# devmentality/LEAStereo

Measured on AMD Instinct MI355X. Metric: stereo pairs/s at 576×960 D=192, 1/2/4/8 GPU; EPE vs reference, higher is better.
Workload: dtype f32; 1 GPU; SceneFlow 576x960 D=192 fp32, batch 1 per GPU (BASELINE configs[1]); height=576, width=960, maxdisp=192, global_batch=1, parallelism=dp1 (pairs sharded over ranks, no collective in the step), launch=hip graph replay

## Files before the change

include/leastereo_hip_tuning.h:

```cpp
#ifndef LEASTEREO_HIP_TUNING_H
#define LEASTEREO_HIP_TUNING_H

#ifdef __cplusplus
extern "C" {
#endif

int lea_conv3d_set_tile_override(int nt, int tw, int td);

int lea_conv3d_set_rs_gather(int on);

int lea_conv1x1_set_vector(int on);

int lea_conv3d_bf16_set_tile_override(int th, int td, int mt);

int lea_conv3d_bf16_set_variant(int variant);

int lea_conv3d_bf16_set_stream1x1(int on);

int lea_conv3d_bf16_set_pair_split(int on);

int lea_resample_bf16_set_batch(int k);

int lea_resample_bf16_set_cols(int on);

int lea_resample_set_mode(int mode);

int lea_conv2d_set_small(int on);

const char* lea_conv2d_kernel_name_cin(int B, int cin, int cout, int H, int W);

int lea_disparity_set_register_form(int on);

int lea_tapsum_set_rows(int on);

int lea_staged_rows(int Hi, int Ho, int ac, int R, int halo);

int lea_conv3d_wino_set_w22(int on);

int lea_conv3d_wino_set_tile_override(int np, int td, int f);

int lea_conv3d_wino_set_variant(int variant);

int lea_conv3d_wino2_set_walk(int spw);

int lea_conv3d_wino2_set_halo16(int on);

int lea_conv3d_wino2_set_lane_halo16(int on);

int lea_conv3d_wino_set_fence(int on);

int lea_conv3d_wino2_set_pipeline(int on);

int lea_conv3d_wino2p_set_wpre(int on);

int lea_conv3d_wino44_set(int on);

int lea_conv3d_wino44_set_upre(int on);

int lea_conv3d_wino44_set_sched(int s);

int lea_conv3d_wino44_set_group(int g);

int lea_conv3d_wino_set_epi_buf(int on);

int lea_conv3d_wino_set_small_cout(int mode);

int lea_conv3d_wino_set_block48(int on);

int lea_rectify_set_tile(int mode);

#ifdef __cplusplus
}
#endif
#endif
```

leastereo_amd/_lib.py:

```python
from __future__ import annotations

import ctypes
import os
import threading

LIB_PATH = os.environ.get(
    "LEASTEREO_HIP_LIB",
    os.path.join(os.path.dirname(os.path.abspath(__file__)), "libleastereo_hip.so"))

ABI_VERSION = 14
LEA_F32 = 0
LEA_BF16 = 1
LEA_RELU = 1
LEA_RESIDUAL = 2
LEA_PAIR_SUM = 4
LEA_CVS_TMAJOR = 8
LEA_E_INVALID = 1001

_p = ctypes.c_void_p
_i = ctypes.c_int
_i64 = ctypes.c_int64
_u = ctypes.c_uint

SIGNATURES = {
# ... 69 lines not shown
    "lea_resample_bf16_set_batch": (_i, [_i]),
    "lea_resample_bf16_set_cols": (_i, [_i]),
    "lea_conv3d_wino_set_w22": (_i, [_i]),
    "lea_conv3d_bf16_set_pair_split": (_i, [_i]),
    "lea_disparity_set_register_form": (_i, [_i]),
    "lea_tapsum_set_rows": (_i, [_i]),
    "lea_staged_rows": (_i, [_i, _i, _i, _i, _i]),
    "lea_conv1x1_resampled_bf16": (_i, [_p, _i64, _i, _i, _i, _p, _p, _p, _p, _i64, _i, _i, _i, _i, _i,
                                        _i, _u, _p]),
    "lea_to_c8_bf16": (_i, [_p, _i64, _p, _i64, _i, _i, _i64, _p]),
    "lea_conv2d_packed_elems_bf16": (ctypes.c_size_t, [_i, _i]),
    "lea_conv2d_pack_weights_bf16": (_i, [_p, _p, _i, _i, _p]),
    "lea_conv2d_bnrelu_bf16": (_i, [_p, _i64, _p, _p, _p, _p, _i64, _p, _i64, _i, _i, _i, _i, _i,
                                    _u, _p]),
    "lea_from_c8_bf16": (_i, [_p, _i64, _p, _i64, _i, _i, _i64, _p]),
    "lea_conv3d_wino_packed_floats": (ctypes.c_size_t, [_i, _i]),
    "lea_conv3d_wino_pack_weights": (_i, [_p, _p, _i, _i, _p]),
    "lea_conv3d_bnrelu_wino": (_i, [_p, _i64, _p, _i64, _i, _p, _p, _p, _p, _i64, _p, _i64,
                                    _i, _i, _i, _i, _i, _i, _u, _i, _p]),
    "lea_conv3d_bnrelu_costvolume_wino": (_i, [_p, _p, _i64, _p, _p, _p, _p, _i64, _i, _i, _i,
                                               _i, _i, _i, _u, _i, _p]),
    "lea_conv3d_wino_kernel_name": (ctypes.c_char_p, [_i, _i, _i, _i, _i, _i, _i]),
    "lea_conv3d_wino_down2_supported": (_i, [_i, _i, _i, _i, _i, _i]),
    "lea_conv3d_wino_down2_kernel_name": (ctypes.c_char_p, [_i, _i, _i, _i, _i, _i]),
    "lea_conv3d_bnrelu_wino_down2": (_i, [_p, _i64, _p, _p, _p, _p, _i64, _i, _i, _i, _i, _i, _i, _u, _i, _p]),
    "lea_conv3d_wino_down2_cat_supported": (_i, [_i, _i, _i, _i, _i, _i, _i]),
    "lea_conv3d_wino_down2_cat_kernel_name": (ctypes.c_char_p, [_i, _i, _i, _i, _i, _i, _i]),
    "lea_conv3d_bnrelu_wino_down2_cat": (_i, [_p, _i64, _p, _i64, _i, _p, _p, _p, _p, _i64, _i, _i, _i, _i, _i, _i,
                                              _u, _i, _p]),
    "lea_conv3d_wino_dp_down2_supported": (_i, [_i, _i, _i, _i, _i, _i]),
    "lea_conv3d_wino_dp_down2_kernel_name": (ctypes.c_char_p, [_i, _i, _i, _i, _i, _i, _i]),
    "lea_conv3d_bnrelu_wino_dp_down2": (_i, [_p, _i64, _p, _p, _p, _p, _i64, _p, _i64, _p, _i64, _i, _i, _i, _i, _i,
                                             _i, _u, _i, _p]),
    "lea_resample3d_down2_supported": (_i, [_i, _i, _i, _i, _i, _i, _i]),
    "lea_resample3d_trilinear_down2": (_i, [_p, _i64, _p, _i64, _p, _i64, _i, _i, _i, _i, _i, _i, _i, _i, _p, _p,
                                            _u, _i, _p]),
    "lea_conv3d_wino_set_tile_override": (_i, [_i, _i, _i]),
    "lea_conv3d_wino_set_variant": (_i, [_i]),
    "lea_conv3d_wino2_set_walk": (_i, [_i]),
    "lea_conv3d_wino2_set_halo16": (_i, [_i]),
    "lea_conv3d_wino2_set_lane_halo16": (_i, [_i]),
    "lea_conv3d_wino_set_fence": (_i, [_i]),
    "lea_resample_set_mode": (_i, [_i]),
    "lea_conv2d_set_small": (_i, [_i]),
    "lea_conv2d_kernel_name_cin": (ctypes.c_char_p, [_i, _i, _i, _i, _i]),
    "lea_conv2d_bnrelu_pair": (_i, [_p, _i64, _p, _p, _p, _p, _i64, _p, _i64, _p, _i64, _i, _i, _i, _i, _i,
                                    _i, _u, _p]),
    "lea_conv3d_wino2_set_pipeline": (_i, [_i]),
    "lea_conv3d_wino2p_set_wpre": (_i, [_i]),
    "lea_conv3d_wino44_set": (_i, [_i]),
    "lea_conv3d_wino44_set_upre": (_i, [_i]),
    "lea_conv3d_wino44_set_sched": (_i, [_i]),
    "lea_conv3d_wino44_set_group": (_i, [_i]),
    "lea_conv3d_wino_set_epi_buf": (_i, [_i]),
    "lea_conv3d_set_rs_gather": (_i, [_i]),
    "lea_conv1x1_set_vector": (_i, [_i]),
    "lea_conv3d_bf16_set_stream1x1": (_i, [_i]),
    "lea_conv3d_wino_set_small_cout": (_i, [_i]),
    "lea_conv3d_wino_set_block48": (_i, [_i]),
    "lea_cv_stem_split_weights": (_i, [_p, _p, _p, _i, _i, _p]),
    "lea_cv_stem_combine": (_i, [_p, _i64, _p, _i64, _p, _p, _p, _i64, _i, _i, _i, _i, _i, _u, _i,
                                 _p]),
    "lea_cv_stem_map_windows": (_i, [_i, _i, ctypes.POINTER(_i), ctypes.POINTER(_i)]),
    "lea_conv2d_windowed_tiles": (_i, [_i, _i, _i, _i, _i, ctypes.POINTER(_i)]),
    "lea_conv2d_bnrelu_windowed": (_i, [_p, _i64, _p, _p, _p, _p, _i64, _i, _i, _i, _i, _i, _i, _i, _i, _i, _i,
                                        _u, _i, _p]),
    "lea_cv_stem_down2_supported": (_i, [_i, _i, _i, _i, _i]),
    "lea_cv_stem_combine_down2": (_i, [_p, _i64, _p, _i64, _p, _p, _p, _i64, _p, _i64, _i, _i, _i, _i, _i,
                                       _u, _i, _p]),
    "lea_standardize_workspace_bytes": (ctypes.c_size_t, [_i]),
    "lea_standardize_crop_u8": (_i, [_p, _p, _i, _i, _i, _i, _p, _p, _i, _i, _p, _p]),
    "lea_train_transform_workspace_bytes": (ctypes.c_size_t, [_i]),
    "lea_train_transform_u8": (_i, [_p, _p, _i, _i, _i, _i, _p, _p, _p, _p, _p, _p, _i, _i,
                                    ctypes.c_float, _p, _p, _p]),
    "lea_standardize_tiles_workspace_bytes": (ctypes.c_size_t, []),
    "lea_standardize_tiles_u8": (_i, [_p, _p, _i, _i, _i, _p, _i, _p, _p, _i, _i, _p, _p]),
    "lea_tile_blend_f32": (_i, [_p, _i64, _p, _i, _p, _i, _i, _i, _i, _i, _i, _i, _i, _p, _i, _i, _p, _p]),
    "lea_disparity_metrics_workspace_bytes": (ctypes.c_size_t, [_i, _i, _i]),
    "lea_disparity_metrics": (_i, [_p, _i64, _p, _i64, _i, _i, _i, ctypes.c_float, _i, _i,
                                   _i, _i, _i, _p, _p, _p, _p]),
    "lea_conv3d_wgrad_workspace_bytes": (ctypes.c_size_t, [_i, _i, _i, _i, _i, _i, _i]),
    "lea_conv3d_wgrad": (_i, [_p, _p, _p, _p, ctypes.c_size_t, _i, _i, _i, _i, _i, _i, _i, _p]),
    "lea_conv2d_wgrad_workspace_bytes": (ctypes.c_size_t, [_i, _i, _i, _i, _i]),
    "lea_conv2d_wgrad": (_i, [_p, _p, _p, _p, ctypes.c_size_t, _i, _i, _i, _i, _i, _p]),
    "lea_conv2d_s3_backward_data": (_i, [_p, _p, _p, _i, _i, _i, _i, _i, _p]),
    "lea_conv2d_s3_wgrad_workspace_bytes": (ctypes.c_size_t, [_i, _i, _i, _i, _i]),
    "lea_conv2d_s3_wgrad": (_i, [_p, _p, _p, _p, ctypes.c_size_t, _i, _i, _i, _i, _i, _p]),
    "lea_conv3d_flip_weights": (_i, [_p, _p, _i, _i, _i, _p]),
    "lea_bn_workspace_bytes": (ctypes.c_size_t, [_i]),
    "lea_bn_forward_f32": (_i, [_p, _p, _i, _i, _i64, _p, _p, _p, _p, ctypes.c_float, ctypes.c_float,
                                _i, _u, _p, _p, _p, _p]),
    "lea_bn_backward_f32": (_i, [_p, _p, _p, _p, _i, _i, _i64, _p, _p, _p, _i, _u, _p, _p, _p, _p]),
    "lea_disparity_regression_backward": (_i, [_p, _p, _p, _p, _i, _i, _i, _i, _i, _p]),
    "lea_build_cost_volume_backward": (_i, [_p, _p, _p, _i, _i, _i, _i, _i, _p]),
    "lea_resample3d_backward_workspace_bytes": (ctypes.c_size_t, [_i, _i, _i, _i, _i, _i, _i, _i]),
    "lea_resample3d_trilinear_backward": (_i, [_p, _p, _p, ctypes.c_size_t, _i, _i, _i, _i, _i, _i, _i, _i,
                                               _i, _p]),
}

_lib = None
_lock = threading.Lock()


class HipKernelError(RuntimeError):
    pass


def load():
    global _lib
    if _lib is not None:
        return _lib
    with _lock:
        if _lib is None:
            if not os.path.exists(LIB_PATH):
                raise HipKernelError(
                    f"{LIB_PATH} not found: build it with `make` (hipcc --offload-arch=gfx950); "
                    "the LEAStereo hot path has no fallback")
            lib = ctypes.CDLL(LIB_PATH)
            for name, (res, args) in SIGNATURES.items():
                fn = getattr(lib, name)
                fn.restype = res
                fn.argtypes = args
            _apply_env_tuning(lib)
            _lib = lib
    return _lib


TUNING_ENV = {"LEASTEREO_WINO2_WALK": "lea_conv3d_wino2_set_walk",
              "LEASTEREO_HALO16": "lea_conv3d_wino2_set_halo16",
              "LEASTEREO_LANE_HALO16": "lea_conv3d_wino2_set_lane_halo16",
              "LEASTEREO_WINO_FENCE": "lea_conv3d_wino_set_fence",
              "LEASTEREO_RESAMPLE_MODE": "lea_resample_set_mode",
              "LEASTEREO_CONV2D_SMALL": "lea_conv2d_set_small",
              "LEASTEREO_WINO2_PIPE": "lea_conv3d_wino2_set_pipeline",
              "LEASTEREO_WINO2P_WPRE": "lea_conv3d_wino2p_set_wpre",
              "LEASTEREO_WINO44": "lea_conv3d_wino44_set",
              "LEASTEREO_WINO44_UPRE": "lea_conv3d_wino44_set_upre",
              "LEASTEREO_EPI_BUF": "lea_conv3d_wino_set_epi_buf",
              "LEASTEREO_RS_GATHER": "lea_conv3d_set_rs_gather",
              "LEASTEREO_1X1_VEC": "lea_conv1x1_set_vector",
              "LEASTEREO_BF16_1X1": "lea_conv3d_bf16_set_stream1x1",
              "LEASTEREO_RESAMPLE_K": "lea_resample_bf16_set_batch",
              "LEASTEREO_RESAMPLE_COLS": "lea_resample_bf16_set_cols",
              "LEASTEREO_W22": "lea_conv3d_wino_set_w22",
              "LEASTEREO_PAIR_SPLIT": "lea_conv3d_bf16_set_pair_split",
              "LEASTEREO_DISP_REG": "lea_disparity_set_register_form",
              "LEASTEREO_TAPSUM_ROWS": "lea_tapsum_set_rows"}


def _apply_env_tuning(lib):
    for var, fn in TUNING_ENV.items():
        if os.environ.get(var):
            if getattr(lib, fn)(int(os.environ[var])) != 0:
                raise HipKernelError(f"{var}={os.environ[var]}: {lib.lea_last_error().decode()}")


def check(rc: int, what: str):
    if rc != 0:
        msg = load().lea_last_error().decode(errors="replace")
        raise HipKernelError(f"{what} failed (rc={rc}): {msg}")
```

leastereo_amd/csrc/conv3d_wino.hip:

```cpp
#include "wino_common.h"

namespace lea {
namespace wino {

template <int F, int Q, int MT, int NP, int TD, bool H16 = false>
struct Cfg {
  static constexpr bool DP = MT == 0;
  static constexpr int MTE = DP ? 1 : MT;
  static constexpr int TDA = DP ? 1 : TD;
  static constexpr int NSTEP = DP ? 12 : 9;
  static_assert(!DP || TD == 2, "a depth-paired tile covers two output planes");
  static constexpr int NX = F + 2;
  static constexpr int COP = 16 * MTE;
  static constexpr bool SWZ = (COP % 32) == 0;
  static constexpr int RPG = 16 / Q;
  static constexpr int TW = F * Q;
  static constexpr int TH = 4 * NP * RPG;
  static constexpr int RH = TH + 2, RW = TW + 2;
  static constexpr int PLANE = RH * RW;
  static constexpr int PLANES = TD + 2;
  static constexpr int IMG = PLANES * PLANE;
  static constexpr int XSLOTS = (IMG + 63) / 64;
  static constexpr int CIS = conflict_free_cis<F, Q>(64 * XSLOTS, RW);
  static constexpr int RWA = TW + 8;
  static constexpr int PLANEA = RH * RWA;
  static constexpr int IMGA = PLANES * PLANEA;
  static constexpr int BLK16 = IMGA / 4;
  static constexpr int PIECES16 = (BLK16 + 63) / 64;
  static constexpr int cb2(int c) {
    int base = 1;
    for (int k = 1; k <= c; ++k) {
      const int want = (k & 1 ? 2 : 0) + (k & 2 ? 32 : 0) + 1, lo = base + IMGA;
      base = lo + ((want - lo) % 64 + 64) % 64;
    }
    return base;
  }
  static_assert(!H16 || (Q == 16 && F == 4), "16-byte halo: one tile row per lane group");
  static constexpr int CSH = PIECES16 * 256;
  static constexpr int cbh(int c) { return 1 + c * CSH; }
  static_assert(!H16 || (CSH % 64 == 0 && RWA % 4 == 0 && PLANEA % 4 == 0), "b128 halo map");
  static constexpr int XS = H16 ? (cbh(CIN_B) + 3) / 4 * 4 : CIN_B * CIS;
  static constexpr int RWX = H16 ? RWA : RW;
  static constexpr int PLX = H16 ? PLANEA : PLANE;
  static constexpr int WS = NSTEP * 3 * CIN_B * COP;
  static constexpr int WSLOTS = (WS + 255) / 256;
  static constexpr int STAGE = XS + 256 * WSLOTS;
  static_assert(XS % 4 == 0 && WS % 4 == 0 && RW % 2 == 0 && PLANE % 2 == 0, "aligned LDS regions and b64 reads");
  static_assert(2 * STAGE * 4 * 2 <= 160 * 1024, "two double-buffered workgroups per CU");
};

constexpr int kDownXch = 4 * 64 * 4;
__device__ __forceinline__ float lerp_dp(float l0, float v0, float l1, float v1) {
// ... 895 lines not shown
    wino::g_override[0] = 0;
    return 0;
  }
  LEA_CHECK_ARG((np == 1 || np == 2) && (td == 1 || td == 2) && (f == 0 || f == 2 || f == 4 || f == 8),
                "lea_conv3d_wino_set_tile_override: bad tile np=%d td=%d f=%d", np, td, f);
  wino::g_override[0] = np;
  wino::g_override[1] = td;
  wino::g_override[2] = f;
  return 0;
}

extern "C" int lea_conv3d_wino_set_block48(int on) {
  clear_error();
  LEA_CHECK_ARG(on == 0 || on == 1, "lea_conv3d_wino_set_block48: on=%d", on);
  wino::g_block48 = on;
  return 0;
}

extern "C" int lea_conv3d_wino_set_epi_buf(int on) {
  clear_error();
  LEA_CHECK_ARG(on == 0 || on == 1, "lea_conv3d_wino_set_epi_buf: on=%d", on);
  wino::g_epibuf = on;
  return 0;
}

extern "C" int lea_conv3d_wino_set_small_cout(int mode) {
  clear_error();
  LEA_CHECK_ARG(mode == 0 || mode == 1, "lea_conv3d_wino_set_small_cout: mode=%d", mode);
  wino::g_small16 = mode;
  return 0;
}

extern "C" int lea_conv3d_wino2_set_pipeline(int on) {
  clear_error();
  LEA_CHECK_ARG(on == 0 || on == 1, "lea_conv3d_wino2_set_pipeline: on=%d", on);
  wino::g_pipe = on;
  return 0;
}

extern "C" int lea_conv3d_wino44_set(int on) {
  clear_error();
  LEA_CHECK_ARG(on >= 0 && on <= 3, "lea_conv3d_wino44_set: on=%d", on);
  wino::g_w44 = on;
  return 0;
}

extern "C" int lea_conv3d_wino44_set_group(int g) {
  clear_error();
  LEA_CHECK_ARG(g >= -1 && g <= 16, "lea_conv3d_wino44_set_group: %d", g);
  wino::g_w44g = g;
  return 0;
}

extern "C" int lea_conv3d_wino44_set_sched(int s) {
  clear_error();
  LEA_CHECK_ARG(s >= 0 && s <= 3, "lea_conv3d_wino44_set_sched: %d", s);
  wino::g_w44s = s;
  return 0;
}

extern "C" int lea_conv3d_wino44_set_upre(int on) {
  clear_error();
  LEA_CHECK_ARG(on == 0 || on == 1, "lea_conv3d_wino44_set_upre: on=%d", on);
  wino::g_w44u = on;
  return 0;
}

extern "C" int lea_conv3d_wino2p_set_wpre(int on) {
  clear_error();
  LEA_CHECK_ARG(on == 0 || on == 1, "lea_conv3d_wino2p_set_wpre: on=%d", on);
  wino::g_wpre = on;
  return 0;
}

extern "C" int lea_conv3d_wino_set_fence(int on) {
  clear_error();
  LEA_CHECK_ARG(on == 0 || on == 1, "lea_conv3d_wino_set_fence: on=%d", on);
  wino::g_fence = on;
  return 0;
}

extern "C" int lea_conv3d_wino2_set_lane_halo16(int on) {
  clear_error();
  LEA_CHECK_ARG(on >= 0 && on <= 2, "lea_conv3d_wino2_set_lane_halo16: on=%d", on);
  wino::g_lane16 = on;
  return 0;
}

extern "C" int lea_conv3d_wino2_set_halo16(int on) {
  clear_error();
  LEA_CHECK_ARG(on == 0 || on == 1, "lea_conv3d_wino2_set_halo16: on=%d", on);
  wino::g_halo16 = on;
  return 0;
}

extern "C" int lea_conv3d_wino2_set_walk(int spw) {
  clear_error();
  LEA_CHECK_ARG(spw >= 0 && spw <= 64, "lea_conv3d_wino2_set_walk: spw=%d", spw);
  wino::g_spw = spw;
  return 0;
}

extern "C" int lea_conv3d_wino_set_w22(int on) {
  clear_error();
  LEA_CHECK_ARG(on >= 0 && on <= 2, "lea_conv3d_wino_set_w22: on=%d", on);
  wino::g_w22 = on;
// ... 307 lines not shown
```

leastereo_amd/csrc/conv3d_wino44.hip:

```cpp
#include <type_traits>

#include "wino_common.h"

namespace lea {
namespace wino {

namespace w44 {
constexpr int Q = 8, F = 4, TW = 32, TH = 2, TD = 4, PLANES = 6, RH = TH + 2, RWA = TW + 8;
constexpr int PLANEA = RH * RWA;
constexpr int BLK16 = PLANES * PLANEA / 4;
constexpr int CB0 = 1, CB1 = CB0 + 1024 + 2, CB2 = CB1 + 1024 + 30, CB3 = CB2 + 1024 + 2;
constexpr int XS = (CB3 + 1024 + 3) / 4 * 4;
constexpr int GS = 40, XHS = 20, TRS = 320, TCS = 1284, TS = 4 * TCS;
constexpr int KGL = 28;
constexpr int KGU = 56;
constexpr int NST = 8;
constexpr int NSTD = 2;
static_assert(CB1 % 64 == 3 && CB2 % 64 == 33 && CB3 % 64 == 35, "V-pass bank map");
static_assert(BLK16 <= 4 * 64 && 4 * 256 <= CB1 - CB0, "whole pieces per channel region");
static_assert(TRS % 64 == 0 && TCS % 8 == 4 && GS % 8 == 0 && XHS % 4 == 0 && TRS >= Q * GS && TCS >= RH * TRS,
              "V bank map");
static_assert(4 * 64 * 20 <= TS && 4 * 64 * 16 <= XS, "epilogue exchange fits a V and a halo buffer");
static_assert((2 * XS + 2 * TS) * 4 * 2 <= 160 * 1024, "two workgroups per CU");
}

__global__ void pack_wino44_lane_kernel(const float* __restrict__ w, float* __restrict__ out, int cout, int cin,
                                        int nchunks, long long total) {
  for (long long i = blockIdx.x * (long long)blockDim.x + threadIdx.x; i < total;
       i += (long long)gridDim.x * blockDim.x) {
    long long q = i;
    const int e = (int)(q % (64 * w44::KGL)); q /= 64 * w44::KGL;
    const int k = (e / 256) * 4 + (e & 3), ln = (e & 255) >> 2;
    const int xh = (int)(q % 2); q /= 2;
    const int wc = (int)(q % 2); q /= 2;
    const int ch = (int)(q % nchunks);
    const int cb = (int)(q / nchunks);
    const int co = cb * 32 + 16 * wc + (ln & 15), c = ch * CIN_B + (ln >> 4);
    float v = 0.f;
    if (k < 27 && co < cout && c < cin) {
      const int kh = k / 9, kd = (k % 9) / 3, x = 3 * xh + k % 3;
      const float* g = w + (((long long)co * cin + c) * 9 + kd * 3 + kh) * 3;
      const float s = g[0] + g[2], s4 = fmaf(4.f, g[2], g[0]);
      const float u[6] = {g[0], s + g[1], s - g[1], fmaf(2.f, g[1], s4), fmaf(-2.f, g[1], s4), g[2]};
      v = u[x];
    }
    out[i] = v;
  }
}

__global__ void pack_wino44_lane_u_kernel(const float* __restrict__ w, float* __restrict__ out, int cout, int cin,
                                          int nchunks, long long total) {
  for (long long i = blockIdx.x * (long long)blockDim.x + threadIdx.x; i < total;
       i += (long long)gridDim.x * blockDim.x) {
    long long q = i;
    const int e = (int)(q % (64 * w44::KGU)); q /= 64 * w44::KGU;
    const int k = (e / 256) * 4 + (e & 3), ln = (e & 255) >> 2;
    const int xh = (int)(q % 2); q /= 2;
    const int wc = (int)(q % 2); q /= 2;
    const int ch = (int)(q % nchunks);
    const int cb = (int)(q / nchunks);
    const int co = cb * 32 + 16 * wc + (ln & 15), c = ch * CIN_B + (ln >> 4);
    float v = 0.f;
    if (k < 54 && co < cout && c < cin) {
      const int kh = k / 18, x = 3 * xh + (k % 18) / 6, ed = k % 6;
      float gwx[3];
      for (int kd = 0; kd < 3; ++kd) {
        const float* g = w + (((long long)co * cin + c) * 9 + kd * 3 + kh) * 3;
        const float s = g[0] + g[2], s4 = fmaf(4.f, g[2], g[0]);
        const float u[6] = {g[0], s + g[1], s - g[1], fmaf(2.f, g[1], s4), fmaf(-2.f, g[1], s4), g[2]};
        gwx[kd] = u[x];
      }
      const float g0 = gwx[0], g1 = gwx[1], g2 = gwx[2];
      const float s = g0 + g2, s4 = fmaf(4.f, g2, g0);
      const float u[6] = {g0, s + g1, s - g1, fmaf(2.f, g1, s4), fmaf(-2.f, g1, s4), g2};
      v = u[ed];
    }
    out[i] = v;
  }
}

long long lane44_g_floats(int cout, int cin) { return (long long)((cout + 31) / 32) * (cin / CIN_B) * 4 * 64 * w44::KGL; }
long long lane44_floats(int cout, int cin) {
  return lane44_g_floats(cout, cin) + (long long)((cout + 31) / 32) * (cin / CIN_B) * 4 * 64 * w44::KGU;
}

namespace {
__device__ __forceinline__ void bt6(const float x0, const float x1, const float x2, const float x3, const float x4,
                                    const float x5, float* v) {
  const float pa = fmaf(-4.f, x2, x4), pb = fmaf(-4.f, x1, x3);
  const float pc = x4 - x2, pd = 2.f * (x3 - x1);
  v[0] = fmaf(4.f, x0, fmaf(-5.f, x2, x4));
  v[1] = pa + pb;
  v[2] = pa - pb;
  v[3] = pc + pd;
  v[4] = pc - pd;
  v[5] = fmaf(4.f, x1, fmaf(-5.f, x3, x5));
}
__device__ __forceinline__ void at6(const float a0, const float a1, const float a2, const float a3, const float a4,
                                    const float a5, float* y) {
  const float m0 = 0.25f * a0;
  const float m1 = (-1.f / 6.f) * a1, m2 = (-1.f / 6.f) * a2;
  const float m3 = (1.f / 24.f) * a3, m4 = (1.f / 24.f) * a4;
  const float sp = m1 + m2, sm = m1 - m2, tp = m3 + m4, tm = m3 - m4;
  y[0] = (m0 + sp) + tp;
  y[1] = fmaf(2.f, tm, sm);
  y[2] = fmaf(4.f, tp, sp);
  y[3] = fmaf(8.f, tm, sm) + a5;
}
}

__device__ __forceinline__ float lerp44(float l0, float v0, float l1, float v1) {
#pragma clang fp contract(off)
  return l0 * v0 + l1 * v1;
}
__device__ __forceinline__ void buf_store2(__amdgpu_buffer_rsrc_t rs, unsigned off, f32x2 v) {
  __builtin_amdgcn_raw_buffer_store_b64(__builtin_bit_cast(u32x2_t, v), rs, off, 0, 0);
}

template <bool UPRE, int SCHED, bool DOWN>
__device__ __forceinline__ void conv3d_wino44_body(const ConvArgs& a) {
  using namespace w44;
  constexpr int NX = 3, NE = 6;
  __shared__ __attribute__((aligned(16))) float smem[2 * XS + 2 * TS];
  const unsigned lds0 = lds_addr(smem);
  float* const halo = smem;
  float* const tvb = smem + 2 * XS;

  const int tid = threadIdx.x;
  const int lane = tid & 63;
  const int wave = __builtin_amdgcn_readfirstlane(tid >> 6);
  const int wc = wave & 1, xh = wave >> 1;
  const int nblk = a.nblk;
  const int xcd = blockIdx.x % 8, idx = blockIdx.x / 8;
  const int q8 = nblk / 8, r8 = nblk % 8;
  const int lin = (xcd < r8 ? xcd * (q8 + 1) : r8 * (q8 + 1) + (xcd - r8) * q8) + idx;
  const int spw = a.spw > 0 ? a.spw : 1;
  const int ngz = (a.ndz + spw - 1) / spw;
  int cob, gz, th, tw, b;
  if (a.grp == 0) {
    cob = lin % a.ncob;
    const int rest = lin / a.ncob;
    gz = rest % ngz;
    const int tile = (rest / ngz) % a.ntiles;
    b = rest / (ngz * a.ntiles);
    th = tile / a.tiles_w;
    tw = tile % a.tiles_w;
  } else {
    const int G = a.grp, nth = a.ntiles / a.tiles_w, ntw = a.tiles_w;
    const int GZ = max(1, 64 / (a.ncob * G * G));
    const int per_b = a.ncob * ngz * a.ntiles;
    b = lin / per_b;
    int r = lin - b * per_b;
    const int slab = a.ncob * GZ * a.ntiles;
    const int i = r / slab;
    r -= i * slab;
    const int cz = min(GZ, ngz - i * GZ);
    const int rowg = a.ncob * cz * G * ntw;
    const int j = r / rowg;
    r -= j * rowg;
    const int ch = min(G, nth - j * G);
    const int cellg = a.ncob * cz * ch * G;
    const int k = r / cellg;
    r -= k * cellg;
    const int cw = min(G, ntw - k * G);
    cob = r % a.ncob;
    r /= a.ncob;
    tw = k * G + r % cw;
    r /= cw;
    th = j * G + r % ch;
    gz = i * GZ + r / ch;
  }
  const int h0 = th * TH;
  const int w0 = tw * TW;
  const int pz0 = gz * spw, nquads = min(spw, a.ndz - pz0);
  const int co0 = cob * 32;
  const int nchunks = a.cin / CIN_B;
  const int nitems = nquads * nchunks;
  const int HW = a.H * a.W;
  const unsigned nrec = (unsigned)(HW * a.D) * 4u;
  const long long cvol = (long long)HW * a.D;
  constexpr int GL = UPRE ? KGU : KGL;
  const float* wl = a.wp + a.uoff + (UPRE ? (long long)a.ncob * nchunks * 4 * 64 * KGL : 0LL) +
                    ((long long)(cob * nchunks) * 4 + wc * 2 + xh) * 64 * GL + lane * 4;

  const int e16 = 64 * wave + lane;
  unsigned hwo16 = 0xFFFFFFF0u;
  int pln16 = -1000;
  {
    const int p = e16 / (RH * (RWA / 4)), r = e16 - p * (RH * (RWA / 4));
    const int rr = r / (RWA / 4), blk = r - rr * (RWA / 4);
    const int h = h0 + rr - 1, w = w0 - 4 + 4 * blk;
    if (e16 < BLK16 && (unsigned)h < (unsigned)a.H && (unsigned)w < (unsigned)a.W) {
      hwo16 = (unsigned)(h * a.W + w) * 4u;
      pln16 = p - 1;
    }
  }
  const unsigned long long cvolb = (unsigned long long)cvol * 4u;
  const unsigned long long xa = (unsigned long long)(a.x + (long long)b * a.xbs);
  const unsigned long long x2s =
      a.x2 ? (unsigned long long)(a.x2 + (long long)b * a.x2bs) - (unsigned long long)a.cin1 * cvolb : xa;
  auto issue_halo = [&](int ch, int qd, int buf) {
    const int d = (pz0 + qd) * TD + pln16;
    const unsigned vo = (hwo16 != 0xFFFFFFF0u && (unsigned)d < (unsigned)a.D)
                            ? hwo16 + (unsigned)d * (unsigned)HW * 4u : 0xFFFFFFF0u;
    const unsigned long long cb = (unsigned long long)(ch * CIN_B) * cvolb;
#pragma unroll
    for (int ci = 0; ci < CIN_B; ++ci) {
      const int c = ch * CIN_B + ci;
      const unsigned long long base = (c < a.cin1 ? xa : x2s) + cb + (unsigned long long)ci * cvolb;
      const __amdgpu_buffer_rsrc_t rs = __builtin_amdgcn_make_buffer_rsrc((void*)base, 0, nrec, 0x00020000);
      constexpr int cbs[4] = {CB0, CB1, CB2, CB3};
      dma_dwordx4_buf(rs, vo, lds0 + 4 * (unsigned)(buf * XS + cbs[ci] + wave * 256));
    }
  };
  float4 gw[GL / 4];
  auto load_g = [&](int ch) {
    const float4* src = reinterpret_cast<const float4*>(wl + (long long)ch * 4 * 64 * GL);
#pragma unroll
    for (int k = 0; k < GL / 4; ++k) gw[k] = src[64 * k];
  };
  const int vg = (tid & 3) | (((tid >> 3) & 1) << 2);
  const int vc = ((tid >> 2) & 1) | (((tid >> 4) & 1) << 1);
  const int vr = (tid >> 5) & 3;
  const int vxh = __builtin_amdgcn_readfirstlane(tid >> 7);
  const int vxo = (vc == 0 ? CB0 : vc == 1 ? CB1 : vc == 2 ? CB2 : CB3) + vr * RWA + 3 + F * vg;
  const int vto = vc * TCS + vr * TRS + GS * vg + XHS * vxh;
  auto vpass = [&](auto XHC, int buf) {
    constexpr int VXH = decltype(XHC)::value;
    const float* sp0 = halo + buf * XS + vxo;
    float bw[PLANES][3];
#pragma unroll
    for (int pl = 0; pl < PLANES; ++pl) {
      const float* sp = sp0 + pl * PLANEA;
      f32x2 a0 = *reinterpret_cast<const f32x2*>(sp);
      f32x2 a1 = *reinterpret_cast<const f32x2*>(sp + 2);
      f32x2 a2 = *reinterpret_cast<const f32x2*>(sp + 4);
      asm volatile("" : "+v"(a0), "+v"(a1), "+v"(a2));
      if constexpr (VXH == 0) {
        const float pa = fmaf(-4.f, a1.x, a2.x), pb = fmaf(-4.f, a0.y, a1.y);
        bw[pl][0] = fmaf(4.f, a0.x, fmaf(-5.f, a1.x, a2.x));
        bw[pl][1] = pa + pb;
        bw[pl][2] = pa - pb;
      } else {
        const float pc = a2.x - a1.x, pd = 2.f * (a1.y - a0.y);
        bw[pl][0] = pc + pd;
        bw[pl][1] = pc - pd;
        bw[pl][2] = fmaf(4.f, a0.y, fmaf(-5.f, a1.y, a2.y));
      }
    }
    float v[3][NE];
#pragma unroll
    for (int x = 0; x < 3; ++x) bt6(bw[0][x], bw[1][x], bw[2][x], bw[3][x], bw[4][x], bw[5][x], v[x]);
    float* tp = tvb + buf * TS + vto;
    const float* vf = &v[0][0];
#pragma unroll
    for (int k = 0; k < 4; ++k)
      *reinterpret_cast<float4*>(tp + 4 * k) = make_float4(vf[4 * k], vf[4 * k + 1], vf[4 * k + 2], vf[4 * k + 3]);
    *reinterpret_cast<f32x4*>(tp + 16) = f32x4{vf[16], vf[17], vf[16], vf[17]};
  };

  const int ci = lane >> 4, p = lane & 15;
  const int pq = p % Q, pr = p / Q;
  const int toff = ci * TCS + pr * TRS + GS * pq + XHS * xh;
  f32x4 acc[NX][NE];
#pragma unroll
  for (int x = 0; x < NX; ++x)
#pragma unroll
    for (int e = 0; e < NE; ++e) acc[x][e] = f32x4{0.f, 0.f, 0.f, 0.f};

  float sc[2], sh[2];
#pragma unroll
  for (int r = 0; r < 2; ++r) {
    const int co = co0 + 16 * wc + 4 * ci + 2 * xh + r;
    const bool cv = co < a.cout;
    sc[r] = (cv && a.scale) ? a.scale[co] : 1.f;
    sh[r] = (cv && a.shift) ? a.shift[co] : 0.f;
  }
  const bool relu = a.flags & LEA_RELU, resid = a.flags & LEA_RESIDUAL;
// ... 209 lines not shown
      };
      auto mfmas = [&](const Xf& T) {
  #pragma unroll
        for (int x = 0; x < NX; ++x)
  #pragma unroll
          for (int e = 0; e < NE; ++e)
            acc[x][e] = __builtin_amdgcn_mfma_f32_16x16x4f32(T.u[x][e], T.v[x][e], acc[x][e], 0, 0, 0);
      };
      Raw raw[2];
      Xf xf[2];
      if constexpr (SCHED != 2) __builtin_amdgcn_iglp_opt(0);
      load_step(0, raw[0]);
      load_step(1, raw[1]);
      xform(0, raw[0], xf[0]);
      issue_halo(hch, hqd, it & 1);
      load_step(2, raw[0]);
      xform(1, raw[1], xf[1]);
      mfmas(xf[0]);
      if constexpr (SCHED == 0 || SCHED == 2) vpass(XHC, (it + 1) & 1);
      xform(2, raw[0], xf[0]);
      load_g(it + 1 < nitems ? (ich + 1 == nchunks ? 0 : ich + 1) : ich);
      mfmas(xf[1]);
      if constexpr (SCHED == 1) vpass(XHC, (it + 1) & 1);
      mfmas(xf[0]);
      if constexpr (SCHED == 3) vpass(XHC, (it + 1) & 1);
      after_epi = false;
      if (ich == nchunks - 1) {
        epilogue_xh(XHC, (pz0 + iqd) * TD, tvb + (it & 1) * TS, halo + ((it + 1) & 1) * XS);
        after_epi = true;
  #pragma unroll
        for (int x = 0; x < NX; ++x)
  #pragma unroll
          for (int e = 0; e < NE; ++e) acc[x][e] = f32x4{0.f, 0.f, 0.f, 0.f};
      }
      if (++ich == nchunks) {
        ich = 0;
        ++iqd;
      }
      if (it + 3 < nitems && ++hch == nchunks) {
        hch = 0;
        ++hqd;
      }
    }
  };
  if (xh == 0)
    run(std::integral_constant<int, 0>{});
  else
    run(std::integral_constant<int, 1>{});
  asm volatile("s_waitcnt vmcnt(0)" ::: "memory");
}

template <bool UPRE, int SCHED>
__global__ __launch_bounds__(256, 2) void conv3d_wino44_kernel(const ConvArgs a) {
  conv3d_wino44_body<UPRE, SCHED, false>(a);
}
__global__ __launch_bounds__(256, 2) void conv3d_wino44_down2_kernel(const ConvArgs a) {
  conv3d_wino44_body<false, 0, true>(a);
}
__global__ __launch_bounds__(256, 2) void conv3d_wino44_down2_cat_kernel(const ConvArgs a) {
  conv3d_wino44_body<false, 0, true>(a);
}

int g_w44 = 2;
int g_w44u = 0;
int g_w44s = 0;
int g_w44g = -1;

int run44(ConvArgs a, int B, int spw, hipStream_t st, bool down) {
  a.ncob = (a.cout + 31) / 32;
  a.tiles_w = (a.W + w44::TW - 1) / w44::TW;
  a.ntiles = a.tiles_w * ((a.H + w44::TH - 1) / w44::TH);
  a.ndz = (a.D + w44::TD - 1) / w44::TD;
  a.spw = std::max(1, std::min(spw > 0 ? spw : auto_walk(a, B, 2), a.ndz));
  const long long n_ = (long long)a.ntiles * ((a.ndz + a.spw - 1) / a.spw) * B * a.ncob;
  LEA_CHECK_ARG(n_ < (1LL << 31), "lea_conv3d(wino44): grid too large");
  a.nblk = (int)n_;
  a.grp = g_w44g >= 0 ? g_w44g : (n_ >= 2048 ? 16 : 0);
  const dim3 grid((unsigned)n_);
  if (down) {
    if (a.x2 && a.cin1 < a.cin)
      conv3d_wino44_down2_cat_kernel<<<grid, 256, 0, st>>>(a);
    else
      conv3d_wino44_down2_kernel<<<grid, 256, 0, st>>>(a);
    return launch_status("lea_conv3d(wino44 down2)");
  }
  if (g_w44u)
    conv3d_wino44_kernel<true, 0><<<grid, 256, 0, st>>>(a);
  else if (g_w44s == 1)
    conv3d_wino44_kernel<false, 1><<<grid, 256, 0, st>>>(a);
  else if (g_w44s == 2)
    conv3d_wino44_kernel<false, 2><<<grid, 256, 0, st>>>(a);
  else if (g_w44s == 3)
    conv3d_wino44_kernel<false, 3><<<grid, 256, 0, st>>>(a);
  else
    conv3d_wino44_kernel<false, 0><<<grid, 256, 0, st>>>(a);
  return launch_status("lea_conv3d(wino44)");
}

}
}
```

leastereo_amd/csrc/wino_common.h:

```cpp
#pragma once
#include "conv3d_impl.h"

namespace lea {
namespace wino {

constexpr int CIN_B = 4;

__host__ __device__ constexpr int mt_of(int cout) {
  return cout <= 8 ? 0 : cout <= 16 ? 1 : (cout % 32 != 0 && cout % 48 == 0) ? 3 : 2;
}
__host__ __device__ constexpr int cop_of(int mt) { return 16 * (mt > 0 ? mt : 1); }

template <int F, int Q>
__host__ __device__ constexpr int lane_dword(int lane, int cis, int rw) {
  return (lane >> 4) * cis + ((lane & 15) / Q) * rw + F * ((lane & 15) % Q);
}
template <int F, int Q>
__host__ __device__ constexpr int conflict_free_cis(int img, int rw) {
  for (int cis = img + (img & 1);; cis += 2) {
    bool used[64] = {};
    bool ok = true;
    for (int l = 0; l < 32 && ok; ++l)
      for (int k = 0; k < 2 && ok; ++k) {
        const int bank = (lane_dword<F, Q>(l, cis, rw) + k) % 64;
// ... 32 lines not shown
typedef unsigned u32x2_t __attribute__((ext_vector_type(2)));
typedef float f32x2 __attribute__((ext_vector_type(2)));
__device__ __forceinline__ __amdgpu_buffer_rsrc_t block_rsrc(const float* base, long long bytes) {
  return __builtin_amdgcn_make_buffer_rsrc((void*)base, 0, (int)(unsigned)bytes, 0x00020000);
}
__device__ __forceinline__ f32x4 buf_load4(__amdgpu_buffer_rsrc_t rs, unsigned off) {
  return __builtin_bit_cast(f32x4, __builtin_amdgcn_raw_buffer_load_b128(rs, off, 0, 0));
}
__device__ __forceinline__ void buf_store4(__amdgpu_buffer_rsrc_t rs, unsigned off, f32x4 v) {
  __builtin_amdgcn_raw_buffer_store_b128(__builtin_bit_cast(u32x4_t, v), rs, off, 0, 0);
}
template <int NST>
__device__ __forceinline__ void wait_item(bool after_epilogue) {
  static_assert(NST > 0 && NST < 64, "vmcnt immediate");
  if (after_epilogue)
    asm volatile("s_waitcnt vmcnt(%0)" ::"n"(NST) : "memory");
  else
    asm volatile("s_waitcnt vmcnt(0)" ::: "memory");
}
inline bool epi_buf_ok(const ConvArgs& a) {
  const long long dhw = (long long)a.D * a.H * a.W;
  bool ok = a.W % 4 == 0 && dhw % 4 == 0 && ((uintptr_t)a.y & 15) == 0 && a.ybs % 4 == 0 &&
            48LL * dhw * 4 < (long long)kEpiOob;
  if (a.flags & LEA_RESIDUAL) ok = ok && ((uintptr_t)a.res & 15) == 0 && a.rbs % 4 == 0;
  return ok;
}

struct Plan2 {
  int q, wc, mte, nw, occ;
  int pv;
  int spw;
};
inline int auto_walk(const ConvArgs& a, int B, int wg_per_cu) {
  const long long base = (long long)a.ntiles * a.ndz * B * a.ncob;
  const long long round = 256LL * wg_per_cu;
  if (a.cin / CIN_B > 16) return 1;
  int s = 1;
  while (s < 4 && base / (2 * s) >= round * 15 / 16) s *= 2;
  return s;
}

int run2(const Plan2& p, ConvArgs a, int B, hipStream_t st, bool cv);
long long lane_weights_floats(int cout, int cin);
long long lane_raw_floats(int cout, int cin);
__global__ void pack_wino_lane_kernel(const float* __restrict__ w, float* __restrict__ out, int cout, int cin,
                                      int nchunks, long long total);
__global__ void pack_wino_lane_wpre_kernel(const float* __restrict__ w, float* __restrict__ out, int cout, int cin,
                                           int nchunks, long long total);
extern int g_wpre;
extern int g_w44;
extern int g_w44u;
extern int g_w44s;
extern int g_w44g;
long long lane44_floats(int cout, int cin);
long long lane44_g_floats(int cout, int cin);
__global__ void pack_wino44_lane_kernel(const float* __restrict__ w, float* __restrict__ out, int cout, int cin,
                                        int nchunks, long long total);
__global__ void pack_wino44_lane_u_kernel(const float* __restrict__ w, float* __restrict__ out, int cout, int cin,
                                          int nchunks, long long total);
int run44(ConvArgs a, int B, int spw, hipStream_t st, bool down = false);
const char* name2(const Plan2& p, bool cv);

long long u22_section(int cout, int cin);
bool wino22_ok(const ConvArgs& a);
int run22(ConvArgs a, int B, int spw, hipStream_t st);
__global__ void pack_wino22_kernel(const float* __restrict__ w, float* __restrict__ out, int cout, int cin,
                                   long long total);

}
}
```

Before: 166.3 pairs/s.

## Add a 16x4 spatial tile variant for the wino44 conv3d kernel

New measurement: 169.1 pairs/s (median of 6 runs). 1.02x the previous value.

```diff
diff --git a/include/leastereo_hip_tuning.h b/include/leastereo_hip_tuning.h
--- a/include/leastereo_hip_tuning.h
+++ b/include/leastereo_hip_tuning.h
@@ -61,6 +61,10 @@
 
 int lea_conv3d_wino44_set_group(int g);
 
+int lea_conv3d_wino44_set_tile(int t);
+
+int lea_conv3d_wino44_tile(int B, int cin, int cout, int D, int H, int W);
+
 int lea_conv3d_wino_set_epi_buf(int on);
 
 int lea_conv3d_wino_set_small_cout(int mode);
diff --git a/leastereo_amd/_lib.py b/leastereo_amd/_lib.py
--- a/leastereo_amd/_lib.py
+++ b/leastereo_amd/_lib.py
@@ -145,6 +145,8 @@
     "lea_conv3d_wino44_set_upre": (_i, [_i]),
     "lea_conv3d_wino44_set_sched": (_i, [_i]),
     "lea_conv3d_wino44_set_group": (_i, [_i]),
+    "lea_conv3d_wino44_set_tile": (_i, [_i]),
+    "lea_conv3d_wino44_tile": (_i, [_i, _i, _i, _i, _i, _i]),
     "lea_conv3d_wino_set_epi_buf": (_i, [_i]),
     "lea_conv3d_set_rs_gather": (_i, [_i]),
     "lea_conv1x1_set_vector": (_i, [_i]),
@@ -229,6 +231,7 @@
               "LEASTEREO_WINO2P_WPRE": "lea_conv3d_wino2p_set_wpre",
               "LEASTEREO_WINO44": "lea_conv3d_wino44_set",
               "LEASTEREO_WINO44_UPRE": "lea_conv3d_wino44_set_upre",
+              "LEASTEREO_WINO44_TILE": "lea_conv3d_wino44_set_tile",
               "LEASTEREO_EPI_BUF": "lea_conv3d_wino_set_epi_buf",
               "LEASTEREO_RS_GATHER": "lea_conv3d_set_rs_gather",
               "LEASTEREO_1X1_VEC": "lea_conv1x1_set_vector",
diff --git a/leastereo_amd/csrc/conv3d_wino.hip b/leastereo_amd/csrc/conv3d_wino.hip
--- a/leastereo_amd/csrc/conv3d_wino.hip
+++ b/leastereo_amd/csrc/conv3d_wino.hip
@@ -1,3 +1,5 @@
+#include <cstring>
+
 #include "wino_common.h"
 
 namespace lea {
@@ -999,6 +1001,20 @@
   return 0;
 }
 
+extern "C" int lea_conv3d_wino44_set_tile(int t) {
+  clear_error();
+  LEA_CHECK_ARG(t == -1 || t == 16 || t == 32, "lea_conv3d_wino44_set_tile: %d", t);
+  wino::g_w44t = t;
+  return 0;
+}
+
+extern "C" int lea_conv3d_wino44_tile(int B, int cin, int cout, int D, int H, int W) {
+  if (cin <= 0 || cin % wino::CIN_B != 0) return 0;
+  const char* name = lea_conv3d_wino_kernel_name(B, cin, cout, D, H, W, 0);
+  if (!name || strcmp(name, "conv3d_wino44_kernel") != 0) return 0;
+  return wino::tile44(B, cin, cout, D, H, W);
+}
+
 extern "C" int lea_conv3d_wino44_set_sched(int s) {
   clear_error();
   LEA_CHECK_ARG(s >= 0 && s <= 3, "lea_conv3d_wino44_set_sched: %d", s);
diff --git a/leastereo_amd/csrc/conv3d_wino44.hip b/leastereo_amd/csrc/conv3d_wino44.hip
--- a/leastereo_amd/csrc/conv3d_wino44.hip
+++ b/leastereo_amd/csrc/conv3d_wino44.hip
@@ -6,22 +6,37 @@
 namespace wino {
 
 namespace w44 {
-constexpr int Q = 8, F = 4, TW = 32, TH = 2, TD = 4, PLANES = 6, RH = TH + 2, RWA = TW + 8;
-constexpr int PLANEA = RH * RWA;
-constexpr int BLK16 = PLANES * PLANEA / 4;
+constexpr int F = 4, TD = 4, PLANES = 6;
 constexpr int CB0 = 1, CB1 = CB0 + 1024 + 2, CB2 = CB1 + 1024 + 30, CB3 = CB2 + 1024 + 2;
 constexpr int XS = (CB3 + 1024 + 3) / 4 * 4;
-constexpr int GS = 40, XHS = 20, TRS = 320, TCS = 1284, TS = 4 * TCS;
+constexpr int GS = 40, XHS = 20;
 constexpr int KGL = 28;
 constexpr int KGU = 56;
 constexpr int NST = 8;
 constexpr int NSTD = 2;
 static_assert(CB1 % 64 == 3 && CB2 % 64 == 33 && CB3 % 64 == 35, "V-pass bank map");
-static_assert(BLK16 <= 4 * 64 && 4 * 256 <= CB1 - CB0, "whole pieces per channel region");
-static_assert(TRS % 64 == 0 && TCS % 8 == 4 && GS % 8 == 0 && XHS % 4 == 0 && TRS >= Q * GS && TCS >= RH * TRS,
-              "V bank map");
-static_assert(4 * 64 * 20 <= TS && 4 * 64 * 16 <= XS, "epilogue exchange fits a V and a halo buffer");
-static_assert((2 * XS + 2 * TS) * 4 * 2 <= 160 * 1024, "two workgroups per CU");
+static_assert(GS % 8 == 0 && XHS % 4 == 0, "V bank map");
+
+template <int Q_>
+struct Geo {
+  static constexpr int Q = Q_, TW = F * Q, TH = 16 / Q, RH = TH + 2, RWA = TW + 8;
+  static constexpr int RSLOTS = Q == 8 ? RH : RH + 1;
+  static constexpr int PLANEA = RSLOTS * RWA;
+  static constexpr int BLK16 = PLANES * PLANEA / 4;
+  static constexpr int TRS = Q * GS, TCS = Q == 8 ? 1284 : 964;
+  static constexpr int TS = 4 * TCS > 4 * 64 * 20 ? 4 * TCS : 4 * 64 * 20;
+  static constexpr int row_slot(int r) { return RSLOTS == RH || r < RH - 1 ? r : r + 1; }
+  static_assert(Q == 8 || Q == 4, "the instantiated geometries");
+  static_assert(BLK16 <= 4 * 64 && 4 * 256 <= CB1 - CB0, "whole pieces per channel region");
+  static_assert(Q == 8 ? TRS % 64 == 0 && TCS % 8 == 4 : TRS % 64 == 32 && TCS % 64 == 4, "V bank map");
+  static_assert(TCS >= RH * TRS, "V rows per channel");
+  static_assert(4 * 64 * 20 <= TS && 4 * 64 * 16 <= XS, "epilogue exchange fits a V and a halo buffer");
+  static_assert((2 * XS + 2 * TS) * 4 * 2 <= 160 * 1024, "two workgroups per CU");
+};
+static_assert((Geo<4>::row_slot(2) - Geo<4>::row_slot(0)) * Geo<4>::RWA % 64 == 48 &&
+                  (Geo<4>::row_slot(3) - Geo<4>::row_slot(1)) * Geo<4>::RWA % 64 == 48 &&
+                  (Geo<4>::row_slot(5) - Geo<4>::row_slot(4)) * Geo<4>::RWA % 64 == 48,
+              "halo row pairs of a V-pass half-wave");
 }
 
 __global__ void pack_wino44_lane_kernel(const float* __restrict__ w, float* __restrict__ out, int cout, int cin,
@@ -117,9 +132,12 @@
   __builtin_amdgcn_raw_buffer_store_b64(__builtin_bit_cast(u32x2_t, v), rs, off, 0, 0);
 }
 
-template <bool UPRE, int SCHED, bool DOWN>
+template <class Geom, bool UPRE, int SCHED, bool DOWN>
 __device__ __forceinline__ void conv3d_wino44_body(const ConvArgs& a) {
   using namespace w44;
+  static_assert(!DOWN || Geom::Q == 8, "the down-sampling epilogue's H partner is lane ^ 8 of the 32 x 2 tile");
+  constexpr int Q = Geom::Q, TW = Geom::TW, TH = Geom::TH, RH = Geom::RH, RWA = Geom::RWA;
+  constexpr int PLANEA = Geom::PLANEA, BLK16 = Geom::BLK16, TRS = Geom::TRS, TCS = Geom::TCS, TS = Geom::TS;
   constexpr int NX = 3, NE = 6;
   __shared__ __attribute__((aligned(16))) float smem[2 * XS + 2 * TS];
   const unsigned lds0 = lds_addr(smem);
@@ -187,10 +205,12 @@
   unsigned hwo16 = 0xFFFFFFF0u;
   int pln16 = -1000;
   {
-    const int p = e16 / (RH * (RWA / 4)), r = e16 - p * (RH * (RWA / 4));
-    const int rr = r / (RWA / 4), blk = r - rr * (RWA / 4);
+    const int p = e16 / (PLANEA / 4), r = e16 - p * (PLANEA / 4);
+    const int rs = r / (RWA / 4), blk = r - rs * (RWA / 4);
+    const int rr = Geom::RSLOTS == RH || rs < RH - 1 ? rs : rs - 1;
+    const bool live = Geom::RSLOTS == RH || rs != RH - 1;
     const int h = h0 + rr - 1, w = w0 - 4 + 4 * blk;
-    if (e16 < BLK16 && (unsigned)h < (unsigned)a.H && (unsigned)w < (unsigned)a.W) {
+    if (live && e16 < BLK16 && (unsigned)h < (unsigned)a.H && (unsigned)w < (unsigned)a.W) {
       hwo16 = (unsigned)(h * a.W + w) * 4u;
       pln16 = p - 1;
     }
@@ -219,11 +239,19 @@
 #pragma unroll
     for (int k = 0; k < GL / 4; ++k) gw[k] = src[64 * k];
   };
-  const int vg = (tid & 3) | (((tid >> 3) & 1) << 2);
-  const int vc = ((tid >> 2) & 1) | (((tid >> 4) & 1) << 1);
-  const int vr = (tid >> 5) & 3;
+  int vg, vc, vr;
+  if constexpr (Q == 8) {
+    vg = (tid & 3) | (((tid >> 3) & 1) << 2);
+    vc = ((tid >> 2) & 1) | (((tid >> 4) & 1) << 1);
+    vr = (tid >> 5) & 3;
+  } else {
+    const int hw = (tid >> 5) & 3, ub = hw == 3 ? 0 : hw, rb = (tid >> 3) & 1;
+    vg = tid & 3;
+    vc = ((tid >> 2) & 1) | (((tid >> 4) & 1) << 1);
+    vr = ub < 2 ? ub + 2 * rb : 4 + rb;
+  }
   const int vxh = __builtin_amdgcn_readfirstlane(tid >> 7);
-  const int vxo = (vc == 0 ? CB0 : vc == 1 ? CB1 : vc == 2 ? CB2 : CB3) + vr * RWA + 3 + F * vg;
+  const int vxo = (vc == 0 ? CB0 : vc == 1 ? CB1 : vc == 2 ? CB2 : CB3) + Geom::row_slot(vr) * RWA + 3 + F * vg;
   const int vto = vc * TCS + vr * TRS + GS * vg + XHS * vxh;
   auto vpass = [&](auto XHC, int buf) {
     constexpr int VXH = decltype(XHC)::value;
@@ -539,24 +567,38 @@
 
 template <bool UPRE, int SCHED>
 __global__ __launch_bounds__(256, 2) void conv3d_wino44_kernel(const ConvArgs a) {
-  conv3d_wino44_body<UPRE, SCHED, false>(a);
+  conv3d_wino44_body<w44::Geo<8>, UPRE, SCHED, false>(a);
+}
+__global__ __launch_bounds__(256, 2) void conv3d_wino44_kernel_16x4(const ConvArgs a) {
+  conv3d_wino44_body<w44::Geo<4>, false, 0, false>(a);
 }
 __global__ __launch_bounds__(256, 2) void conv3d_wino44_down2_kernel(const ConvArgs a) {
-  conv3d_wino44_body<false, 0, true>(a);
+  conv3d_wino44_body<w44::Geo<8>, false, 0, true>(a);
 }
 __global__ __launch_bounds__(256, 2) void conv3d_wino44_down2_cat_kernel(const ConvArgs a) {
-  conv3d_wino44_body<false, 0, true>(a);
+  conv3d_wino44_body<w44::Geo<8>, false, 0, true>(a);
 }
 
 int g_w44 = 2;
 int g_w44u = 0;
 int g_w44s = 0;
 int g_w44g = -1;
+int g_w44t = -1;
+
+int tile44(int B, int cin, int cout, int D, int H, int W) {
+  (void)B, (void)cin, (void)cout, (void)D, (void)H;
+  if (g_w44u || g_w44s != 0) return 32;
+  if (g_w44t > 0) return g_w44t;
+  auto padded = [&](int tw) { return (W + tw - 1) / tw * tw; };
+  return padded(w44::Geo<4>::TW) < padded(w44::Geo<8>::TW) ? 16 : 32;
+}
 
 int run44(ConvArgs a, int B, int spw, hipStream_t st, bool down) {
+  const bool narrow = !down && tile44(B, a.cin, a.cout, a.D, a.H, a.W) == 16;
+  const int tw = narrow ? w44::Geo<4>::TW : w44::Geo<8>::TW, th = narrow ? w44::Geo<4>::TH : w44::Geo<8>::TH;
   a.ncob = (a.cout + 31) / 32;
-  a.tiles_w = (a.W + w44::TW - 1) / w44::TW;
-  a.ntiles = a.tiles_w * ((a.H + w44::TH - 1) / w44::TH);
+  a.tiles_w = (a.W + tw - 1) / tw;
+  a.ntiles = a.tiles_w * ((a.H + th - 1) / th);
   a.ndz = (a.D + w44::TD - 1) / w44::TD;
   a.spw = std::max(1, std::min(spw > 0 ? spw : auto_walk(a, B, 2), a.ndz));
   const long long n_ = (long long)a.ntiles * ((a.ndz + a.spw - 1) / a.spw) * B * a.ncob;
@@ -571,7 +613,9 @@
       conv3d_wino44_down2_kernel<<<grid, 256, 0, st>>>(a);
     return launch_status("lea_conv3d(wino44 down2)");
   }
-  if (g_w44u)
+  if (narrow)
+    conv3d_wino44_kernel_16x4<<<grid, 256, 0, st>>>(a);
+  else if (g_w44u)
     conv3d_wino44_kernel<true, 0><<<grid, 256, 0, st>>>(a);
   else if (g_w44s == 1)
     conv3d_wino44_kernel<false, 1><<<grid, 256, 0, st>>>(a);
diff --git a/leastereo_amd/csrc/wino_common.h b/leastereo_amd/csrc/wino_common.h
--- a/leastereo_amd/csrc/wino_common.h
+++ b/leastereo_amd/csrc/wino_common.h
@@ -108,6 +108,8 @@
 extern int g_w44u;
 extern int g_w44s;
 extern int g_w44g;
+extern int g_w44t;
+int tile44(int B, int cin, int cout, int D, int H, int W);
 long long lane44_floats(int cout, int cin);
 long long lane44_g_floats(int cout, int cin);
 __global__ void pack_wino44_lane_kernel(const float* __restrict__ w, float* __restrict__ out, int cout, int cin,
```
